# soham2560/MPCHoloNavigation

Hardware: AMD Instinct MI355X
Metric: rollouts/sec per computeVelocityCommands() tick (higher is better)
Workload: dtype f32

## Files before the change

### mpcholonavigation_amd/csrc/smpc_api.cpp

```cpp

#include "smpc_ctx.h"

#include <emmintrin.h>

namespace smpc_impl {

thread_local std::string g_create_error;

int fail(smpc_ctx* c, int code, const std::string& msg)
{
  if (c) c->err = msg; else g_create_error = msg;
  return code;
}

int wait_map_upload(smpc_ctx* c)
{
  if (!c->map_pending) return SMPC_OK;
  HIPCK(c, hipEventSynchronize(c->ev_map));
  c->map_pending = false;
  return SMPC_OK;
}

void bar_copy(void* dev_dst, const void* host_src, size_t n)
{
// ... 291 lines not shown
int update_time_major(smpc_ctx* c)
{
  if (!c->use_tpr) return SMPC_OK;
  const uint32_t B = c->cfg.batch_size, T = c->cfg.time_steps;
  HIPCK(c, smpc_launch_relayout(c->d_nvx, c->d_tvx, B, T, true, c->stream));
  HIPCK(c, smpc_launch_relayout(c->d_nvy, c->d_tvy, B, T, true, c->stream));
  HIPCK(c, smpc_launch_relayout(c->d_nwz, c->d_twz, B, T, true, c->stream));
  return SMPC_OK;
}

int ensure_row_major(smpc_ctx* c)
{
  if (c->rm_valid) return SMPC_OK;
  const uint32_t B = c->cfg.batch_size, T = c->cfg.time_steps;
  HIPCK(c, smpc_launch_relayout(c->d_tvx, c->d_nvx, B, T, false, c->stream));
  if (c->holonomic) HIPCK(c, smpc_launch_relayout(c->d_tvy, c->d_nvy, B, T, false, c->stream));
  HIPCK(c, smpc_launch_relayout(c->d_twz, c->d_nwz, B, T, false, c->stream));
  c->rm_valid = true;
  return SMPC_OK;
}

static int launch_draw(smpc_ctx* c, float* nvx, float* nvy, float* nwz, float* tvx, float* tvy, float* twz,
                       hipStream_t st, bool* rm_valid_out)
{
  const uint64_t n = static_cast<uint64_t>(c->cfg.batch_size) * c->cfg.time_steps;
  const uint64_t base = c->cfg.shard_offset * c->cfg.time_steps;
  const uint32_t B = c->cfg.batch_size, T = c->cfg.time_steps;
  if (c->use_tpr && (T & 3u) == 0 && !getenv("SMPC_NO_FUSED_FILL")) {
    HIPCK(c, smpc_launch_fill_noise_tm(tvx, B, T, base, c->seed, 0, c->epoch, c->cfg.vx_std, st));
    HIPCK(c, smpc_launch_fill_noise_tm(twz, B, T, base, c->seed, 1, c->epoch, c->cfg.wz_std, st));
    if (c->holonomic)
      HIPCK(c, smpc_launch_fill_noise_tm(tvy, B, T, base, c->seed, 2, c->epoch, c->cfg.vy_std, st));
    else
      HIPCK(c, hipMemsetAsync(tvy, 0, static_cast<size_t>(SMPC_GM_ROLLOUTS(B)) * T * sizeof(float), st));
    *rm_valid_out = false;
    return SMPC_OK;
  }
  HIPCK(c, smpc_launch_fill_noise(nvx, n, base, c->seed, 0, c->epoch, c->cfg.vx_std, st));
  HIPCK(c, smpc_launch_fill_noise(nwz, n, base, c->seed, 1, c->epoch, c->cfg.wz_std, st));
  if (c->holonomic) HIPCK(c, smpc_launch_fill_noise(nvy, n, base, c->seed, 2, c->epoch, c->cfg.vy_std, st));
  if (c->use_tpr) {
    HIPCK(c, smpc_launch_relayout(nvx, tvx, B, T, true, st));
    HIPCK(c, smpc_launch_relayout(nvy, tvy, B, T, true, st));
    HIPCK(c, smpc_launch_relayout(nwz, twz, B, T, true, st));
  }
  *rm_valid_out = true;
  return SMPC_OK;
}

int cancel_redraw(smpc_ctx* c)
{
  if (!c->redraw_pending) return SMPC_OK;
  HIPCK(c, hipEventSynchronize(c->ev_fill));
  c->redraw_pending = false;
  return SMPC_OK;
}

int absorb_redraw(smpc_ctx* c)
{
  if (!c->redraw_pending) return SMPC_OK;
  HIPCK(c, hipStreamWaitEvent(c->stream, c->ev_fill, 0));
  std::swap(c->d_nvx, c->b_nvx);
  std::swap(c->d_nvy, c->b_nvy);
  std::swap(c->d_nwz, c->b_nwz);
  std::swap(c->d_tvx, c->b_tvx);
  std::swap(c->d_tvy, c->b_tvy);
  std::swap(c->d_twz, c->b_twz);
  c->rm_valid = c->redraw_rm_valid;
  c->redraw_pending = false;
  c->noise_gen++;
  return SMPC_OK;
}

int draw_noise(smpc_ctx* c)
{
  int rc = cancel_redraw(c);
  if (rc != SMPC_OK) return rc;
  bool rm = true;
  rc = launch_draw(c, c->d_nvx, c->d_nvy, c->d_nwz, c->d_tvx, c->d_tvy, c->d_twz, c->stream, &rm);
  if (rc != SMPC_OK) return rc;
  HIPCK(c, hipStreamSynchronize(c->stream));
  c->have_noise = true;
  c->rm_valid = rm;
  c->noise_gen++;
  return SMPC_OK;
}

int redraw_async(smpc_ctx* c)
{
  if (c->redraw_pending) return SMPC_OK;
  const size_t n = static_cast<size_t>(c->cfg.batch_size) * c->cfg.time_steps * sizeof(float);
  if (!c->fill_stream) {
    HIPCK(c, hipStreamCreateWithFlags(&c->fill_stream, hipStreamNonBlocking));
    HIPCK(c, hipEventCreateWithFlags(&c->ev_fill, hipEventDisableTiming));
  }
  if (c->use_tpr && !c->b_tvx) {
    const size_t ngm = static_cast<size_t>(SMPC_GM_ROLLOUTS(c->cfg.batch_size)) * c->cfg.time_steps * sizeof(float);
    HIPCK(c, hipMalloc(&c->b_tvx, 3 * ngm));
    c->b_tvy = c->b_tvx + ngm / sizeof(float);
    c->b_twz = c->b_tvy + ngm / sizeof(float);
  }
  if (!c->b_nvx) {
    HIPCK(c, hipMalloc(&c->b_nvx, n));
    HIPCK(c, hipMalloc(&c->b_nvy, n));
    HIPCK(c, hipMalloc(&c->b_nwz, n));
    if (!c->holonomic) HIPCK(c, hipMemset(c->b_nvy, 0, n));
  }
  c->epoch++;
  bool rm = true;
  const int rc = launch_draw(c, c->b_nvx, c->b_nvy, c->b_nwz, c->b_tvx, c->b_tvy, c->b_twz, c->fill_stream, &rm);
  if (rc != SMPC_OK) return rc;
  HIPCK(c, hipEventRecord(c->ev_fill, c->fill_stream));
  c->redraw_rm_valid = rm;
  c->redraw_pending = true;
  return SMPC_OK;
}

static Knobs read_knobs()
{
  Knobs k;
  auto set = [](const char* name) {return getenv(name) != nullptr;};
  auto number = [](const char* name, int unset) {const char* e = getenv(name); return e ? atoi(e) : unset;};
  if (const char* e = getenv("SMPC_PASS"))
    k.pass = !strcmp(e, "wave") ? Knobs::kWave : !strcmp(e, "lane") ? Knobs::kLane : !strcmp(e, "split") ? Knobs::kSplit : Knobs::kAuto;
  k.no_split = set("SMPC_NO_SPLIT");
  k.split_nseg = static_cast<uint32_t>(std::max(0, number("SMPC_SPLIT_NSEG", 0)));
  k.lane_reread = number("SMPC_LANE_REREAD", 0) != 0;
  k.half_blocks = !set("SMPC_NO_HALF_BLOCKS");
  k.max_blocks_per_cu = static_cast<uint32_t>(std::max(0, number("SMPC_MAX_BLOCKS_PER_CU", 0)));
  k.balanced_grid = !set("SMPC_NO_BALANCED_GRID");
  k.fused_reduce = set("SMPC_FUSED_REDUCE");
// ... 126 lines not shown
  c->stream = c->own_stream;
  if (getenv("SMPC_LANE_TIMELINE")) {
    static_assert(SMPC_TAIL_STAMPS_AT == 8192 + kMaxGrid * 8, "the tail's stamps sit behind the lane pass's");
    CK(hipMalloc(&c->d_timeline, (SMPC_SCAN_COUNT_AT + kMaxGrid * 8) * sizeof(unsigned long long)));
    CK(hipMemset(c->d_timeline, 0, (SMPC_SCAN_COUNT_AT + kMaxGrid * 8) * sizeof(unsigned long long)));
  }
  CK(hipEventCreate(&c->ev0));
  CK(hipEventCreateWithFlags(&c->ev_map, hipEventDisableTiming));
  CK(hipEventCreate(&c->ev1));
  for (auto& e : c->evp) CK(hipEventCreate(&e));
  const uint32_t T = cfg->time_steps;
  c->R = T <= 64 ? 1 : (T <= 128 ? 2 : 4);
  const size_t n = static_cast<size_t>(cfg->batch_size) * T * sizeof(float);
  CK(hipMalloc(&c->d_nvx, n));
  CK(hipMalloc(&c->d_nvy, n));
  if (!c->holonomic) CK(hipMemset(c->d_nvy, 0, n));
  CK(hipMalloc(&c->d_nwz, n));
  {
    bool tpr = cfg->batch_size >= kLaneMinBatch && cfg->time_steps <= kLaneMaxT;
    if (cfg->time_steps <= 64 && cfg->time_steps >= 36 && (cfg->time_steps & 3u) == 0 && cfg->batch_size >= kSplitMinBatch &&
        !c->knobs.no_split)
      tpr = true;
    if (cfg->flags & SMPC_FLAG_WAVE_PER_ROLLOUT) tpr = false;
    if (cfg->flags & SMPC_FLAG_LANE_PER_ROLLOUT) {
      tpr = true;
      c->lane_forced = true;
    }
    if (c->knobs.pass == Knobs::kWave) tpr = false;
    if (c->knobs.pass == Knobs::kLane || c->knobs.pass == Knobs::kSplit) {
      tpr = true;
      c->lane_forced = true;
    }
    if (cfg->flags & SMPC_FLAG_STORE_TRAJECTORIES) tpr = false;
    const size_t ngm = static_cast<size_t>(SMPC_GM_ROLLOUTS(cfg->batch_size)) * T * sizeof(float);
    if (3ull * ngm >= (1ull << 32)) tpr = false;
    c->use_tpr = tpr;
    if (tpr) {
      CK(hipMalloc(&c->d_tvx, 3 * ngm));
      c->d_tvy = c->d_tvx + ngm / sizeof(float);
      c->d_twz = c->d_tvy + ngm / sizeof(float);
      if (!c->holonomic) CK(hipMemset(c->d_tvy, 0, ngm));
      CK(lane_set_lds_limit(static_cast<int>(kLdsPerCu)));
      CK(split_set_lds_limit(static_cast<int>(kLdsPerCu)));
    }
  }
  CK(hipMalloc(&c->d_costs[0], cfg->batch_size * sizeof(float)));
  CK(hipMalloc(&c->d_costs[1], cfg->batch_size * sizeof(float)));
  CK(hipMemset(c->d_costs[0], 0, cfg->batch_size * sizeof(float)));
  CK(hipMemset(c->d_costs[1], 0, cfg->batch_size * sizeof(float)));
  if (cfg->flags & SMPC_FLAG_STORE_TRAJECTORIES) {
    for (int i = 0; i < 3; ++i) {
      CK(hipMalloc(&c->d_traj[i], n));
      CK(hipMemset(c->d_traj[i], 0, n));
    }
  }
  c->tick_cap = tick_layout(T, SMPC_MAX_PATH).total;
  CK(hipMalloc(&c->d_tick, c->tick_cap));
  CK(hipHostMalloc(&c->h_tick, c->tick_cap, hipHostMallocDefault));
  CK(hipMalloc(&c->d_lut, 256 * sizeof(SmpcLut)));
  CK(hipMemset(c->d_lut, 0, 256 * sizeof(SmpcLut)));
  CK(hipMalloc(&c->d_lut_fp, 512 * sizeof(SmpcLut)));
  CK(hipMemset(c->d_lut_fp, 0, 512 * sizeof(SmpcLut)));
  CK(hipHostMalloc(&c->h_lut_fp, 512 * sizeof(SmpcLut), hipHostMallocDefault));
  CK(hipHostMalloc(&c->h_lut, 256 * sizeof(SmpcLut), hipHostMallocDefault));
  const size_t TL = 4 + 3 * static_cast<size_t>(T);
  CK(hipMalloc(&c->d_partials, (kMaxGrid * TL + 16) * sizeof(float)));
  CK(hipMemset(c->d_partials, 0, (kMaxGrid * TL + 16) * sizeof(float)));
  CK(hipMalloc(&c->d_tuple, TL * sizeof(float)));
  CK(hipMalloc(&c->d_out, (3 * T + 8) * sizeof(float)));
  CK(hipMalloc(&c->d_u_iter, 3 * T * sizeof(float)));
  CK(hipHostMalloc(&c->h_out, (3 * T + 8 + kPollWords) * sizeof(float), hipHostMallocMapped));
  memset(c->h_out, 0, (3 * T + 8 + kPollWords) * sizeof(float));
  CK(hipHostGetDevicePointer(reinterpret_cast<void**>(&c->h_out_dev), c->h_out, 0));
  CK(hipMalloc(&c->d_furthest, 32));
// ... 605 lines not shown
```

### mpcholonavigation_amd/csrc/smpc_dev.h

```cpp
#ifndef SMPC_DEV_H_
#define SMPC_DEV_H_

#include <stdint.h>

#define SD_OBSTACLES 0x001u
#define SD_PATH_ALIGN 0x002u
#define SD_PATH_FOLLOW 0x004u
#define SD_GOAL_ANGLE 0x008u
#define SD_PREFER_FORWARD 0x010u
#define SD_USE_PATH_YAW 0x020u
#define SD_ACCUMULATE 0x040u
#define SD_STORE_TRAJ 0x080u
#define SD_TRACK_UNKNOWN 0x100u
#define SD_NEED_FURTHEST 0x200u
#define SD_LOCAL_FURTHEST 0x400u
#define SD_CONSTRAINT 0x800u
#define SD_COST 0x1000u
#define SD_GOAL 0x2000u
#define SD_TWIRLING 0x4000u
#define SD_PATH_ANGLE 0x8000u
#define SD_DEADBAND 0x10000u
#define SD_FP_OBSTACLES 0x20000u
#define SD_FP_COST 0x40000u
#define SD_PATH_ALIGN_LEGACY 0x80000u
#define SD_PAL_USE_PATH_YAW 0x100000u
#define SD_EXTRA_CRITICS (SD_CONSTRAINT | SD_COST | SD_GOAL | SD_TWIRLING | SD_PATH_ANGLE | SD_DEADBAND | \
                          SD_FP_OBSTACLES | SD_FP_COST | SD_PATH_ALIGN_LEGACY)

#define SMPC_GM_ROLLOUTS(B) ((((B) + 63u) / 64u) * 64u)
#define SMPC_GM_INDEX(b, t, T) ((((size_t)(b) >> 6) * (T) + (t)) * 64u + ((b) & 63u))

#define SMPC_MAX_PATH 1024
#define SMPC_MAX_R 4

struct SmpcLut {
  float crit;
  float rep;
};

struct SmpcFinal {
  int enabled;
  float vx_max, vx_min, vy_max, wz_max;
  float* u_dev;
  float* u_host;
  const float* furthest_used;
  uint32_t* done_counter;
  uint32_t seq;
};

struct SmpcDev {
  uint32_t B, T, P;
  uint32_t nsamp;
  uint32_t step;
  uint32_t flags;
  double x0, y0;
  float yaw0, cos0, sin0;
  float svx, svy, swz;
  float dt;
  const float* nvx;
  const float* nvy;
  const float* nwz;
  const float* tvx;
  const float* tvy;
// ... 174 lines not shown
```

### mpcholonavigation_amd/csrc/smpc_kernels.hip

```cpp

#include <hip/hip_runtime.h>
#include <stdio.h>
#include <algorithm>
#include <stdint.h>

#include "smpc_dev.h"
#include "smpc_device_math.h"
#include "smpc_tail.h"
#include "smpc_inst.h"

#define WAVE 64

template <int CTRL, int ROW_MASK = 0xF>
__device__ __forceinline__ float dpp_f(float old, float v)
{
  return __int_as_float(__builtin_amdgcn_update_dpp(__float_as_int(old), __float_as_int(v), CTRL,
                                                    ROW_MASK, 0xF, false));
}
template <int CTRL, int ROW_MASK = 0xF>
__device__ __forceinline__ uint32_t dpp_u(uint32_t old, uint32_t v)
{
  return (uint32_t)__builtin_amdgcn_update_dpp((int)old, (int)v, CTRL, ROW_MASK, 0xF, false);
}

// ... 1308 lines not shown
                                                      float sigma)
{
  const uint64_t q_first = base >> 2;
  const uint64_t q_last = (base + n + 3) >> 2;
  for (uint64_t q = q_first + (uint64_t)blockIdx.x * blockDim.x + threadIdx.x; q < q_last;
       q += (uint64_t)gridDim.x * blockDim.x) {
    uint32_t r[4];
    philox4x32_10((uint32_t)q, (uint32_t)(q >> 32), stream, epoch, (uint32_t)seed,
                  (uint32_t)(seed >> 32), r);
    float z[4];
    box_muller(r[0], r[1], z[0], z[1]);
    box_muller(r[2], r[3], z[2], z[3]);
    const uint64_t e0 = q << 2;
#pragma unroll
    for (int k = 0; k < 4; ++k) {
      const uint64_t e = e0 + (uint64_t)k;
      if (e >= base && e < base + n) out[e - base] = z[k] * sigma;
    }
  }
}

__global__ void __launch_bounds__(256) smpc_fill_noise_tm(float* __restrict__ dst, uint32_t B, uint32_t T,
                                                         uint64_t base, uint64_t seed, uint32_t stream,
                                                         uint32_t epoch, float sigma)
{
  const uint32_t tq = blockIdx.y;
  for (uint32_t b = blockIdx.x * blockDim.x + threadIdx.x; b < B; b += gridDim.x * blockDim.x) {
    const uint64_t q = (base + (uint64_t)b * T + 4u * tq) >> 2;
    uint32_t r[4];
    philox4x32_10((uint32_t)q, (uint32_t)(q >> 32), stream, epoch, (uint32_t)seed, (uint32_t)(seed >> 32), r);
    float z[4];
    box_muller(r[0], r[1], z[0], z[1]);
    box_muller(r[2], r[3], z[2], z[3]);
#pragma unroll
    for (int k = 0; k < 4; ++k) dst[SMPC_GM_INDEX(b, 4u * tq + (uint32_t)k, T)] = z[k] * sigma;
  }
}

__global__ void smpc_sincos_kernel(const float* __restrict__ x, uint32_t n,
                                   float* __restrict__ sn, float* __restrict__ cs)
{
  const uint32_t i = blockIdx.x * blockDim.x + threadIdx.x;
  if (i < n) {
    float s, c;
    smpc_sincos(x[i], s, c);
    sn[i] = s;
    cs[i] = c;
  }
}

hipError_t smpc_launch_sincos(const float* x, uint32_t n, float* sn, float* cs, hipStream_t st)
{
  hipLaunchKernelGGL(smpc_sincos_kernel, dim3((n + 255) / 256), dim3(256), 0, st, x, n, sn, cs);
  return hipGetLastError();
}

__global__ void smpc_philox_kernel(const uint32_t* __restrict__ ctr, uint32_t k0, uint32_t k1, uint32_t n,
                                   uint32_t* __restrict__ out)
{
  const uint32_t i = blockIdx.x * blockDim.x + threadIdx.x;
  if (i < n) {
    uint32_t r[4];
    philox4x32_10(ctr[4 * i], ctr[4 * i + 1], ctr[4 * i + 2], ctr[4 * i + 3], k0, k1, r);
#pragma unroll
    for (int k = 0; k < 4; ++k) out[4 * i + k] = r[k];
  }
}

// ... 139 lines not shown
```

### mpcholonavigation_amd/csrc/smpc_lane.hip

```cpp

#include <hip/hip_runtime.h>
#include <stdint.h>
#include <stdio.h>

#include <type_traits>

#include "smpc_dev.h"
#include "smpc_device_math.h"
#include "smpc_tail.h"
#include "smpc_lane_common.h"
#include "smpc_inst.h"

#ifndef WAVE
#define WAVE 64
#endif
#define LANE_BLOCK 512
#define LANE_BLOCK_RR 512

template <bool TO_GM>
__global__ void __launch_bounds__(256) smpc_relayout(const float* __restrict__ src, float* __restrict__ dst,
                                                    uint32_t B, uint32_t T)
{
  __shared__ float tile[32][33];
  const uint32_t b0 = blockIdx.x * 32, t0 = blockIdx.y * 32;
  const uint32_t lx = threadIdx.x & 31, ly = threadIdx.x >> 5;
  if (TO_GM) {
    for (uint32_t k = ly; k < 32; k += 8) {
      const uint32_t b = b0 + k, t = t0 + lx;
      tile[k][lx] = (b < B && t < T) ? src[(size_t)b * T + t] : 0.f;
    }
    __syncthreads();
    for (uint32_t k = ly; k < 32; k += 8) {
      const uint32_t t = t0 + k, b = b0 + lx;
      if (b < B && t < T) dst[SMPC_GM_INDEX(b, t, T)] = tile[lx][k];
    }
  } else {
    for (uint32_t k = ly; k < 32; k += 8) {
      const uint32_t t = t0 + k, b = b0 + lx;
      tile[lx][k] = (b < B && t < T) ? src[SMPC_GM_INDEX(b, t, T)] : 0.f;
    }
    __syncthreads();
    for (uint32_t k = ly; k < 32; k += 8) {
      const uint32_t b = b0 + k, t = t0 + lx;
      if (b < B && t < T) dst[(size_t)b * T + t] = tile[k][lx];
    }
  }
}

hipError_t smpc_launch_relayout(const float* src, float* dst, uint32_t B, uint32_t T, bool to_gm, hipStream_t st)
{
  const dim3 grid((B + 31) / 32, (T + 31) / 32);
  if (to_gm) hipLaunchKernelGGL(smpc_relayout<true>, grid, dim3(256), 0, st, src, dst, B, T);
  else hipLaunchKernelGGL(smpc_relayout<false>, grid, dim3(256), 0, st, src, dst, B, T);
  return hipGetLastError();
}

__global__ void __launch_bounds__(64) smpc_lane_reduce_kernel(const float* __restrict__ v,
                                                              const float* __restrict__ w,
                                                              float* __restrict__ out)
{
  const int lane = threadIdx.x;
  float V[64];
#pragma unroll
  for (int t = 0; t < 64; ++t) V[t] = v[lane * 64 + t];
  const LaneW lw = lane_weights(w[lane], lane);
  out[lane] = lane_reduce64(V, lw, lane);
}

hipError_t smpc_launch_lane_reduce(const float* v, const float* w, float* out, hipStream_t st)
{
  hipLaunchKernelGGL(smpc_lane_reduce_kernel, dim3(1), dim3(64), 0, st, v, w, out);
  return hipGetLastError();
// ... 132 lines not shown
```

### mpcholonavigation_amd/csrc/smpc_lane_pass.inc

```
template <bool FULL, bool OBST, bool MANY, int NCH, bool RR, bool GA = false, bool QUADS = FULL, int TC = 0, bool DEP = false>
__global__ void __launch_bounds__(RR ? LANE_BLOCK_RR : LANE_BLOCK, 1)
LANE_PASS_KERNEL(const SmpcDev p0, const SmpcLds L, const SmpcDev* __restrict__ many)
{
  constexpr bool POW = LANE_PASS_POW;
  constexpr bool NH = LANE_PASS_NH;
  static_assert(!NH || (OBST && !MANY && !RR && !GA && !DEP && !POW && NCH == 1 && QUADS),
                "no vy stream: the plain ObstaclesCritic rows of whole quads only");
  static_assert(RR || NCH == 1, "parked controls: one chunk of 64 steps");
  static_assert(!POW || (!MANY && !RR && !DEP), "cost powers: the single-context parking form of the five critics");
  static_assert(!FULL || QUADS, "T == 64 is a multiple of four");
  static_assert(TC == 0 || (!FULL && QUADS && !RR && TC < 64 && (TC & 3) == 0), "compile-time horizon: whole quads below 64");
  static_assert(!DEP || (OBST && !RR && !GA), "deployed-list instances: parking form");
  const SmpcDev& p = MANY ? many[blockIdx.y] : p0;
  const SmpcTickPtrs tk{p.u, p.px, p.py, p.pyaw, p.D, p.pf_idx, p.pvalid, p.pa_active, p.pang_active, p.pal_active};
  extern __shared__ __attribute__((aligned(16))) unsigned char smem[];
  uint8_t* s_map = smem;
  const SmpcLut* s_lut = reinterpret_cast<const SmpcLut*>(smem + L.off_lut);
  float* s_px = reinterpret_cast<float*>(smem + L.off_px);
  float* s_py = reinterpret_cast<float*>(smem + L.off_py);
  float* s_D = reinterpret_cast<float*>(smem + L.off_D) + 1;
  f32x4* s_pts4 = reinterpret_cast<f32x4*>(smem + L.off_pts4);
  float* s_su2 = reinterpret_cast<float*>(smem + L.off_scr) - 4;
  constexpr bool kPrune = !GA && !DEP && !MANY && !RR && !POW;
  float* s_prune = reinterpret_cast<float*>(smem + L.off_prune);
// ... 64 lines not shown
      float a = 0.f, b = 0.f, c = 0.f;
      const uint32_t Tn = FULL ? 64u * NCH : (TC ? (uint32_t)TC : p.T);
      for (uint32_t t = (uint32_t)tid; t < Tn; t += WAVE) {
        const float ux = tk.u[t], uy = NH ? 0.f : tk.u[Tn + t], uz = tk.u[2 * Tn + t];
        a = fmaf(ux, ux, a);
        b = fmaf(uy, uy, b);
        c = fmaf(uz, uz, c);
      }
      for (int o = 32; o > 0; o >>= 1) {
        a += __shfl_xor(a, o, WAVE);
        b += __shfl_xor(b, o, WAVE);
        c += __shfl_xor(c, o, WAVE);
      }
      if (tid == 0) {
        s_su2[0] = a;
        s_su2[1] = b;
        s_su2[2] = c;
      }
    }
    for (uint32_t i = tid + blk; i < p.P; i += blk) {
      const float qx = tk.px[i], qy = tk.py[i];
      const bool seg = i + 1 < p.P;
      s_px[i] = qx;
      s_py[i] = qy;
      if (seg) s_D[i] = tk.D[i];
      s_pts4[i] = f32x4{qx, qy, (seg && tk.pvalid[i]) ? 1.0f : 0.f, 0.f};
    }
  }
  __syncthreads();
  stamp(1);

  const cfloat_p cu = (cfloat_p)(uintptr_t)p.u;
  const uint32_t T = FULL ? 64u * NCH : (TC ? (uint32_t)TC : p.T), B = p.B;
  const uint32_t noise_bytes = T * SMPC_GM_ROLLOUTS(B) * 4u;
  const __amdgpu_buffer_rsrc_t rn = __builtin_amdgcn_make_buffer_rsrc(const_cast<float*>(p.tvx), 0, 3u * noise_bytes, 0x00020000);
  const float dt = p.dt, yaw0 = p.yaw0;
  const double x0 = p.x0, y0 = p.y0;
  uint32_t S = 0;
  if (p.flags & SD_NEED_FURTHEST) {
    S = p.d_furthest ? smpc_furthest_index(*p.d_furthest) : p.furthest_hint;
    if (S >= p.P) S = p.P ? p.P - 1 : 0;
  }
  if (lane == 0) {
    s_D[-1] = -3.0e38f;
    s_D[S] = 3.0e38f;
  }
  const bool pa_on = (p.flags & SD_PATH_ALIGN) && p.P > 0 && tk.pa_active[S] && S > 0;
  float pf_x = 0.f, pf_y = 0.f;
  if ((p.flags & SD_PATH_FOLLOW) && p.P > 0) {
    const uint32_t idx = tk.pf_idx[S];
    pf_x = tk.px[idx];
    pf_y = tk.py[idx];
  }
  const uint32_t bs_iters = S > 1 ? 32u - (uint32_t)__builtin_clz(S - 1) : 0u;
  float pa_inv_spacing = 0.f;
  if (pa_on && S > 1 && tk.D[S - 1] > 0.f) pa_inv_spacing = (float)(S - 1) / tk.D[S - 1];
  const bool want_local_furthest = (p.flags & SD_NEED_FURTHEST) && (p.flags & SD_LOCAL_FURTHEST);
  const bool con_on = DEP && (p.flags & SD_CONSTRAINT) != 0, tw_on = DEP && (p.flags & SD_TWIRLING) != 0;
  const float k_con = p.dt * p.con_weight, k_tw = p.tw_weight / (float)(FULL ? 64 * NCH : (TC ? TC : (int)p.T));
  const bool cost_mode = DEP && (p.flags & SD_COST) != 0;
  constexpr bool ga_on = GA;
  const uint32_t nquad = (T + 3u) >> 2;

  float m_run = 3.0e38f, s_run = 0.f;
  float Ux[NCH], Uy[NCH], Uz[NCH];
#pragma unroll
  for (int h = 0; h < NCH; ++h) Ux[h] = Uy[h] = Uz[h] = 0.f;
// ... 13 lines not shown
    const bool live = b < B;
    const uint32_t bl = live ? b : B - 1;
    f32x32 PX0, PX1, PY0, PY1;
    if constexpr (NH) {
      if (!FULL) PX0 = PX1 = (f32x32)(0.f);
    } else if (!FULL && !RR) PX0 = PX1 = PY0 = PY1 = (f32x32)(0.f);

    float cpx = p.svx, cpy = NH ? 0.f : p.svy, cpz = p.swz;
    float acc_yaw = 0.f, ax = 0.f, ay = 0.f;
    float cs_prev = p.cos0, sn_prev = p.sin0;
    float x = 0.f, y = 0.f;
    float crit = 0.f, rep = 0.f;
    float yaw_max = 0.f;
    float alive = 1.0f;
    uint32_t cell_q = 256u;
    f32x2 e_q = {0.f, 0.f};
    auto lookup_wait = [&]() {};
    auto lookup_accumulate = [&]() {
      alive = e_q.x < 0.f ? 0.f : alive;
      crit = fmaf(alive, e_q.x, crit);
      rep = fmaf(alive, e_q.y, rep);
    };
    auto lookup_issue_entry = [&]() {
      const SmpcLut e = s_lut[cell_q];
      e_q = f32x2{e.crit, e.rep};
    };
    auto lookup_issue_byte = [&](uint32_t idx) {cell_q = s_map[idx];};
    float pfw = 0.f, gx = 0.f, gy = 0.f, gz = 0.f;
    float ga_sum = 0.f;
    float ext = 0.f;
    float traj_dist = 0.f, pa_sum = 0.f, pa_num = 0.f, sx_prev = p.x00f, sy_prev = p.y00f;
    uint32_t path_pt = 0;

    const float k_rinv = p.rinvf, k_cx = p.cxf, k_cy = p.cyf;
    const float k_edge = 0.5f - p.cell_eps_w;
    auto do_step = [&](const uint32_t t, const bool sample_slot, const float ux, const float uy, const float uz,
                       const float n0, const float n1, const float n2, float& cvx, float& cvy,
                       float& cwz) __attribute__((always_inline)) {
      cvx = ux + n0;
      if constexpr (!NH) cvy = uy + n1;
      cwz = uz + n2;
      const float vx = cpx, vy = cpy, wz = cpz;
      cpx = cvx;
      if constexpr (!NH) cpy = cvy;
      cpz = cwz;
      acc_yaw = acc_yaw + wz * dt;
      const float yaw = acc_yaw + yaw0;
      const float dxr = NH ? vx * cs_prev : vx * cs_prev - vy * sn_prev;
      const float dyr = NH ? vx * sn_prev : vx * sn_prev + vy * cs_prev;
      ax = ax + dxr * dt;
      ay = ay + dyr * dt;
      if constexpr (DEP) {
        if (con_on) {
          const float sp = fast_sqrt(vx * vx + vy * vy);
          const float vt = vx > 0.f ? sp : -sp;
          const float e = fmaxf(vt - p.con_max_vel, 0.f) + fmaxf(p.con_min_vel - vt, 0.f);
          ext = fmaf(e, k_con, ext);
        }
        if (tw_on) ext = fmaf(fabsf(wz), k_tw, ext);
      }
      if (ga_on) {
        const float a = p.ga_goal_yaw - yaw;
        const float kf = fmaf(a, 0.15915494309189535f, 12582912.0f);
        const float k = kf - 12582912.0f;
        float r = fmaf(-k, 6.2831854820251465f, a);
        r = fmaf(-k, -1.7484555e-07f, r);
        ga_sum += fabsf(r);
      }

      uint32_t idx = 0;
      if (OBST) {
        const float qx = fmaf(ax, k_rinv, k_cx), qy = fmaf(ay, k_rinv, k_cy);
        const float rx = __builtin_amdgcn_fractf(qx), ry = __builtin_amdgcn_fractf(qy);
        const int lx = cvt_floor_i32(qx), ly = cvt_floor_i32(qy);
// ... 36 lines not shown
        uint32_t lo = gi + (c1 ? 1u : 0u);
        float dl = c1 ? db : da, dh = c1 ? dc : db;
        if (__builtin_expect(__builtin_amdgcn_ballot_w64(!c0 || c2) != 0, 0)) {
          uint32_t base = 0, nn = S;
          for (uint32_t it = 0; it < bs_iters; ++it) {
            const uint32_t half = nn >> 1;
            base = (s_D[base + half - 1 + (half == 0)] < dist && half) ? base + half : base;
            nn -= half;
          }
          const float d_base = s_D[base];
          lo = base + (d_base < dist ? 1u : 0u);
          dl = lo > 0 ? s_D[lo - 1] : 0.f;
          dh = lo < S ? s_D[lo] : 0.f;
        }
        uint32_t pt;
        if (lo == path_pt) pt = 0;
        else if (lo >= S) pt = S - 1;
        else pt = (dist - dl < dh - dist) ? lo - 1 : lo;
        path_pt = pt;
        const f32x4 q = s_pts4[pt];
        const float ex = q[0] - x, ey = q[1] - y;
        const float d = fast_sqrt(ex * ex + ey * ey);
        pa_num += q[2];
        pa_sum = fmaf(q[2], d, pa_sum);
      }
      if (OBST) {
        lookup_wait();
        lookup_accumulate();
        lookup_issue_entry();
        lookup_issue_byte(idx);
      }
    };

    const uint32_t loff = ((bl >> 6) * T * 64u + (bl & 63u)) * 4u;
    constexpr uint32_t step_bytes = 256u;
    auto ld = [&](uint32_t tensor, uint32_t t) -> float {
      const uint32_t tc = (FULL || t < T) ? t : T - 1;
      return __uint_as_float(__builtin_amdgcn_raw_buffer_load_b32(rn, loff, tensor * noise_bytes + tc * step_bytes, 0));
    };
    auto ldu = [&](uint32_t ctrl, uint32_t t) -> float {return cu[ctrl * T + ((FULL || t < T) ? t : T - 1)];};
    float nq[12], uq[12];
#pragma unroll
    for (int i = 0; i < 4; ++i) {
      nq[3 * i + 0] = ld(0, i);
      if constexpr (!NH) nq[3 * i + 1] = ld(1, i);
      nq[3 * i + 2] = ld(2, i);
#pragma unroll
      for (int k = 0; k < 3; ++k) {
        if constexpr (NH) {
          if (k == 1) continue;
        }
        uq[3 * i + k] = ldu(k, i);
      }
    }
    uint64_t clk = __builtin_amdgcn_s_memtime();
    auto run_quad = [&](auto hi_c, auto swap_c, const uint32_t q, float (&cq)[12]) __attribute__((always_inline)) {
      constexpr bool SWAP = decltype(swap_c)::value;
      if constexpr (SWAP) {
        __builtin_amdgcn_s_setprio(0);
        if (((uint32_t)(clk >> 15) + (uint32_t)(wave >> 2)) & 1u) __builtin_amdgcn_s_setprio(1);
        clk = __builtin_amdgcn_s_memtime();
      }
      float uc[12];
#pragma unroll
      for (int j = 0; j < 12; ++j) {
        if constexpr (NH) {
          if (j % 3 == 1) continue;
        }
        uc[j] = uq[j];
      }
      constexpr bool kAlwaysAhead = !FULL && TC == 0;
      if (kAlwaysAhead || q + 1 < nquad) {
#pragma unroll
        for (int i = 0; i < 4; ++i)
#pragma unroll
          for (int k = 0; k < 3; ++k) {
            if constexpr (NH) {
              if (k == 1) continue;
            }
            uq[3 * i + k] = ldu(k, 4 * (q + 1) + i);
          }
      }
      constexpr bool kQuadOff = QUADS && !GA && !DEP && !MANY && !POW;
#pragma unroll
      for (int i = 0; i < 4; ++i) {
        const uint32_t t = 4 * q + i;
        const float n0 = nq[3 * i], n1 = NH ? 0.f : nq[3 * i + 1], n2 = nq[3 * i + 2];
        if (kAlwaysAhead || q + 1 < nquad) {
          if constexpr (kQuadOff) {
            const uint32_t tq = (FULL || TC || 4 * (q + 1) < T) ? 4 * (q + 1) : T - 4;
            const uint32_t so0 = tq * step_bytes, so1 = noise_bytes + so0, so2 = noise_bytes + so1;
            auto ldq = [&](uint32_t so) -> float {
              return __uint_as_float(__builtin_amdgcn_raw_buffer_load_b32(rn, loff + (uint32_t)i * step_bytes, so, 0));
            };
            nq[3 * i + 0] = ldq(so0);
            if constexpr (!NH) nq[3 * i + 1] = ldq(so1);
            nq[3 * i + 2] = ldq(so2);
          } else {
            nq[3 * i + 0] = ld(0, t + 4);
            nq[3 * i + 1] = ld(1, t + 4);
            nq[3 * i + 2] = ld(2, t + 4);
          }
        }
        cq[3 * i] = cq[3 * i + 1] = cq[3 * i + 2] = 0.f;
        if (QUADS || t < T)
          do_step(t, i == 0, uc[3 * i], NH ? 0.f : uc[3 * i + 1], uc[3 * i + 2], n0, n1, n2, cq[3 * i], cq[3 * i + 1],
                  cq[3 * i + 2]);
      }
    };
    constexpr bool kPairLoops = FULL || TC != 0;
#define LANE_PARK_QUAD(HI, Q) \
      if constexpr (!RR) { \
        _Pragma("unroll") for (int i = 0; i < 4; ++i) { \
          if constexpr (HI) { \
            PX1[8 * i + ((Q) - 8)] = cq[3 * i]; \
            if constexpr (!NH) PY1[8 * i + ((Q) - 8)] = cq[3 * i + 1]; \
          } else { \
            PX0[8 * i + (Q)] = cq[3 * i]; \
            if constexpr (!NH) PY0[8 * i + (Q)] = cq[3 * i + 1]; \
          } \
          park[(4 * (Q) + i) * LANE_PARK_STRIDE + lane] = cq[3 * i + 2]; \
        } \
      }
    if constexpr (kPairLoops) {
#define LANE_QUAD(HI, SWAP, Q) \
    { \
      float cq[12]; \
      run_quad(std::bool_constant<HI>{}, std::bool_constant<SWAP>{}, (Q), cq); \
      LANE_PARK_QUAD(HI, Q) \
    }
#define LANE_QUADS(HI, Q0, QE)    \
    { \
      uint32_t q = (Q0); \
      const uint32_t qe = (QE); \
      for (; q + 1 < qe; q += 2) { \
        LANE_QUAD(HI, true, q) \
        LANE_QUAD(HI, false, q + 1) \
// ... 117 lines not shown
        uni += p.pf_weight * fast_sqrt(fdx * fdx + fdy * fdy);
      }
      if (p.flags & SD_PREFER_FORWARD) lin += (pfw * -dt) * p.pfw_weight;
      if (ga_on) uni += (ga_sum / (float)T) * p.ga_weight;
      lin += p.g_vx * (gx - s_su2[0]);
      lin += p.g_wz * (gz - s_su2[2]);
      if constexpr (!NH) lin += p.g_vy * (gy - s_su2[1]);
      cost += uni + lin;
      if (pa_on) {
        const float c_pa = pa_num > 0.f ? pa_sum * fast_rcp(pa_num) : 0.f;
        cost += c_pa * p.pa_weight;
      }
    }
    if (live) p.costs[b] = cost;

    float cmin = live ? cost : 3.0e38f;
    for (int o = 32; o > 0; o >>= 1) cmin = fminf(cmin, __shfl_xor(cmin, o, WAVE));
    const float m_new = fminf(m_run, cmin);
    const float f = __builtin_amdgcn_exp2f(p.k2 * (m_run - m_new));
    const float w = live ? __builtin_amdgcn_exp2f(p.k2 * (cost - m_new)) : 0.f;
    float wsum = w;
    for (int o = 32; o > 0; o >>= 1) wsum += __shfl_xor(wsum, o, WAVE);
    s_run = fmaf(s_run, f, wsum);
    m_run = m_new;

    const LaneW lw = lane_weights(w, lane);
    if constexpr (RR) {
#pragma unroll
      for (int h = 0; h < NCH; ++h) {
#pragma unroll
        for (int ctrl = 0; ctrl < 3; ++ctrl) {
          float V[64];
#pragma unroll
          for (int t = 0; t < 64; ++t) V[t] = ld(ctrl, 64u * h + t);
          __builtin_amdgcn_sched_barrier(0);
#pragma unroll
          for (int t = 0; t < 64; ++t) {
            const uint32_t tt = 64u * h + t;
            const float c = ldu(ctrl, tt) + V[t];
            V[t] = (FULL || tt < T) ? c : 0.f;
          }
          const float r = lane_reduce64(V, lw, lane);
          if (ctrl == 0) Ux[h] = fmaf(Ux[h], f, r);
          else if (ctrl == 1) Uy[h] = fmaf(Uy[h], f, r);
          else Uz[h] = fmaf(Uz[h], f, r);
        }
      }
    } else {
      {
        float V[64];
#pragma unroll
        for (int t = 0; t < 32; ++t) {
          V[t] = PX0[8 * (t & 3) + (t >> 2)];
          V[32 + t] = PX1[8 * (t & 3) + (t >> 2)];
        }
        Ux[0] = fmaf(Ux[0], f, lane_reduce64(V, lw, lane));
        if constexpr (!NH) {
#pragma unroll
          for (int t = 0; t < 32; ++t) {
            V[t] = PY0[8 * (t & 3) + (t >> 2)];
            V[32 + t] = PY1[8 * (t & 3) + (t >> 2)];
          }
          Uy[0] = fmaf(Uy[0], f, lane_reduce64(V, lw, lane));
        }
      }
      {
        s_w[lane] = w;
// ... 84 lines not shown
```

### mpcholonavigation_amd/csrc/smpc_split.hip

```cpp

#include <hip/hip_runtime.h>
#include <stdint.h>
#include <stdio.h>

#include "smpc_dev.h"
#include "smpc_device_math.h"
#include "smpc_lane_common.h"
#include "smpc_inst.h"

#define SPLIT_BLOCK 512

typedef const float __attribute__((address_space(4))) * cfloat_ps;
typedef float f32x16 __attribute__((ext_vector_type(16)));
typedef float f32x8 __attribute__((ext_vector_type(8)));
template <int N> struct vecN;
template <> struct vecN<32> {typedef f32x32 type;};
template <> struct vecN<16> {typedef f32x16 type;};
template <> struct vecN<8> {typedef f32x8 type;};
template <> struct vecN<4> {typedef f32x4 type;};

template <int N, int K, int Rr>
__device__ __forceinline__ float row_reduce_node(const float (&V)[N], int lane)
{
  if constexpr ((64 >> K) == N) {
// ... 134 lines not shown
      if (seg_on) s_D[tid] = g_D;
      s_pts4[tid] = f32x4{g_px, g_py, g_valid ? 1.0f : 0.f, 0.f};
    }
    for (uint32_t i = tid + blk; i < p.P; i += blk) {
      const float qx = tk.px[i], qy = tk.py[i];
      const bool seg = i + 1 < p.P;
      s_px[i] = qx;
      s_py[i] = qy;
      if (seg) s_D[i] = tk.D[i];
      s_pts4[i] = f32x4{qx, qy, (seg && tk.pvalid[i]) ? 1.0f : 0.f, 0.f};
    }
    if (tid < 3 * 64) s_u[tid] = g_u;
    if (tid < WAVE) {
      const bool in = (uint32_t)tid < T;
      float a = in ? tk.u[tid] : 0.f, b = in ? tk.u[T + tid] : 0.f, c = in ? tk.u[2 * T + tid] : 0.f;
      a *= a;
      b *= b;
      c *= c;
      for (int o = 32; o > 0; o >>= 1) {
        a += __shfl_xor(a, o, WAVE);
        b += __shfl_xor(b, o, WAVE);
        c += __shfl_xor(c, o, WAVE);
      }
      if (tid == 0) {
        s_su2[0] = a;
        s_su2[1] = b;
        s_su2[2] = c;
      }
    }
  }
  __syncthreads();

  const uint32_t B = p.B;
  const uint32_t noise_bytes = T * SMPC_GM_ROLLOUTS(B) * 4u;
  const __amdgpu_buffer_rsrc_t rn = __builtin_amdgcn_make_buffer_rsrc(const_cast<float*>(p.tvx), 0, 3u * noise_bytes, 0x00020000);
  constexpr uint32_t row_bytes = 256u;
  const float dt = p.dt, yaw0 = p.yaw0;
  const double x0 = p.x0, y0 = p.y0;
  uint32_t S = 0;
  if (p.flags & SD_NEED_FURTHEST) {
    S = p.d_furthest ? smpc_furthest_index(*p.d_furthest) : p.furthest_hint;
    if (S >= p.P) S = p.P ? p.P - 1 : 0;
  }
  if (lane == 0) {
    s_D[-1] = -3.0e38f;
    s_D[S] = 3.0e38f;
  }
  const bool pa_on = (p.flags & SD_PATH_ALIGN) && p.P > 0 && tk.pa_active[S] && S > 0;
  float pf_x = 0.f, pf_y = 0.f;
  if ((p.flags & SD_PATH_FOLLOW) && p.P > 0) {
    const uint32_t idx = tk.pf_idx[S];
    pf_x = tk.px[idx];
    pf_y = tk.py[idx];
  }
  const uint32_t bs_iters = S > 1 ? 32u - (uint32_t)__builtin_clz(S - 1) : 0u;
  float pa_inv_spacing = 0.f;
  if (pa_on && S > 1 && tk.D[S - 1] > 0.f) pa_inv_spacing = (float)(S - 1) / tk.D[S - 1];
  const bool want_local_furthest = (p.flags & SD_NEED_FURTHEST) && (p.flags & SD_LOCAL_FURTHEST);
  const float k_rinv = p.rinvf, k_cx = p.cxf, k_cy = p.cyf;
  const float k_edge = 0.5f - p.cell_eps_w;

  float m_run = 3.0e38f, s_run = 0.f;
  float Ux = 0.f, Uy = 0.f, Uz = 0.f;
  float F_local = 0.f;
  uint32_t n_noncoll = 0;

  const uint32_t ngroups = (B + SPLIT_ROLL - 1) / SPLIT_ROLL;
  const uint32_t gw = blockIdx.x * nwave + wave;
  const uint32_t nW = gridDim.x * nwave;
  const uint32_t t0 = (uint32_t)sg * SPLIT_SEG;

  for (uint32_t grp = gw; grp < ngroups; grp += nW) {
    const uint32_t b = grp * SPLIT_ROLL + (uint32_t)r;
    const bool live = b < B;
    const uint32_t bl = live ? b : B - 1;
    const uint32_t voff = ((bl >> 6) * T * 64u + (bl & 63u)) * 4u + t0 * row_bytes;
    const uint32_t vprev = sg ? voff - row_bytes : voff;
    auto ld = [&](uint32_t tensor, uint32_t i) -> float {
      return __uint_as_float(__builtin_amdgcn_raw_buffer_load_b32(rn, voff, tensor * noise_bytes + i * row_bytes, 0));
    };
    auto ld_prev = [&](uint32_t tensor) -> float {
      return __uint_as_float(__builtin_amdgcn_raw_buffer_load_b32(rn, vprev, tensor * noise_bytes, 0));
    };
    const float* ux_s = s_u + t0;
    const float* uy_s = s_u + 64 + t0;
    const float* uz_s = s_u + 128 + t0;
    auto act = [&](int i) -> bool {return FULL || t0 + (uint32_t)i < T;};

    float ya[SPLIT_SEG];
    float wprev;
    {
      float nz[SPLIT_SEG];
      const float nzp = ld_prev(2);
#pragma unroll
      for (int i = 0; i < SPLIT_SEG; ++i) nz[i] = ld(2, i);
      const float uzp = s_u[128 + (sg ? t0 - 1 : 0)];
      wprev = sg ? uzp + nzp : p.swz;
      float acc = 0.f, w = wprev;
#pragma unroll
      for (int i = 0; i < SPLIT_SEG; ++i) {
        acc = acc + w * dt;
        ya[i] = acc;
        w = act(i) ? uz_s[i] + nz[i] : 0.f;
        park[i * WAVE + lane] = w;
      }
    }
    const float yaw_off = seg_exclusive<NSEG>(ya[SPLIT_SEG - 1], r, sg);

    constexpr int Q = SPLIT_SEG / 4;
#define SLOT(i) (Q * ((i) & 3) + ((i) >> 2))
    typename vecN<SPLIT_SEG>::type cvx;
    float cvy[PARK_VY ? 1 : SPLIT_SEG];
    typename vecN<SPLIT_SEG>::type AX, AY;
    float vxp, vyp;
    {
      const float nxp = ld_prev(0), nyp = ld_prev(1);
      float ny[SPLIT_SEG];
#pragma unroll
      for (int i = 0; i < SPLIT_SEG; ++i) {
        cvx[SLOT(i)] = ld(0, i);
        ny[i] = ld(1, i);
      }
      vxp = sg ? s_u[t0 - 1] + nxp : p.svx;
      vyp = sg ? s_u[64 + t0 - 1] + nyp : p.svy;
#pragma unroll
      for (int i = 0; i < SPLIT_SEG; ++i) {
        cvx[SLOT(i)] = act(i) ? ux_s[i] + cvx[SLOT(i)] : 0.f;
        ny[i] = act(i) ? uy_s[i] + ny[i] : 0.f;
        if constexpr (PARK_VY) park_y[i * WAVE + lane] = ny[i];
        else cvy[i] = ny[i];
      }
      float cs_prev = p.cos0, sn_prev = p.sin0;
      if (sg) smpc_sincos(yaw_off + yaw0, sn_prev, cs_prev);
      float ax = 0.f, ay = 0.f;
#pragma unroll
      for (int i = 0; i < SPLIT_SEG; ++i) {
        const float vx = i ? cvx[SLOT(i - 1)] : vxp, vy = i ? ny[i - 1] : vyp;
        const float dxr = vx * cs_prev - vy * sn_prev;
        const float dyr = vx * sn_prev + vy * cs_prev;
        ax = ax + dxr * dt;
        ay = ay + dyr * dt;
        AX[SLOT(i)] = ax;
        AY[SLOT(i)] = ay;
        if (i + 1 < SPLIT_SEG) smpc_sincos((yaw_off + ya[i]) + yaw0, sn_prev, cs_prev);
      }
    }
    const float x_off = seg_exclusive<NSEG>(AX[SLOT(SPLIT_SEG - 1)], r, sg);
    const float y_off = seg_exclusive<NSEG>(AY[SLOT(SPLIT_SEG - 1)], r, sg);

    float crit = 0.f, rep = 0.f, alive = 1.0f;
    float pfw = 0.f, gx = 0.f, gy = 0.f, gz = 0.f;
    typename vecN<NSAMP>::type sxv, syv;
    float x_end = 0.f, y_end = 0.f;
    float vx_state = vxp;
// ... 338 lines not shown
```

Baseline: 5.765 billion.

## Interleave noise tensors in groups of four timesteps for 128-bit loads

```diff
diff --git a/mpcholonavigation_amd/csrc/smpc_api.cpp b/mpcholonavigation_amd/csrc/smpc_api.cpp
--- a/mpcholonavigation_amd/csrc/smpc_api.cpp
+++ b/mpcholonavigation_amd/csrc/smpc_api.cpp
@@ -347,7 +347,7 @@
     if (c->holonomic)
       HIPCK(c, smpc_launch_fill_noise_tm(tvy, B, T, base, c->seed, 2, c->epoch, c->cfg.vy_std, st));
     else
-      HIPCK(c, hipMemsetAsync(tvy, 0, static_cast<size_t>(SMPC_GM_ROLLOUTS(B)) * T * sizeof(float), st));
+      HIPCK(c, hipMemsetAsync(tvy, 0, SMPC_GM_ELEMS(B, T) * sizeof(float), st));
     *rm_valid_out = false;
     return SMPC_OK;
   }
@@ -410,8 +410,9 @@
     HIPCK(c, hipEventCreateWithFlags(&c->ev_fill, hipEventDisableTiming));
   }
   if (c->use_tpr && !c->b_tvx) {
-    const size_t ngm = static_cast<size_t>(SMPC_GM_ROLLOUTS(c->cfg.batch_size)) * c->cfg.time_steps * sizeof(float);
+    const size_t ngm = SMPC_GM_ELEMS(c->cfg.batch_size, c->cfg.time_steps) * sizeof(float);
     HIPCK(c, hipMalloc(&c->b_tvx, 3 * ngm));
+    HIPCK(c, hipMemset(c->b_tvx, 0, 3 * ngm));
     c->b_tvy = c->b_tvx + ngm / sizeof(float);
     c->b_twz = c->b_tvy + ngm / sizeof(float);
   }
@@ -604,14 +605,14 @@
       c->lane_forced = true;
     }
     if (cfg->flags & SMPC_FLAG_STORE_TRAJECTORIES) tpr = false;
-    const size_t ngm = static_cast<size_t>(SMPC_GM_ROLLOUTS(cfg->batch_size)) * T * sizeof(float);
+    const size_t ngm = SMPC_GM_ELEMS(cfg->batch_size, T) * sizeof(float);
     if (3ull * ngm >= (1ull << 32)) tpr = false;
     c->use_tpr = tpr;
     if (tpr) {
       CK(hipMalloc(&c->d_tvx, 3 * ngm));
       c->d_tvy = c->d_tvx + ngm / sizeof(float);
       c->d_twz = c->d_tvy + ngm / sizeof(float);
-      if (!c->holonomic) CK(hipMemset(c->d_tvy, 0, ngm));
+      CK(hipMemset(c->d_tvx, 0, 3 * ngm));
       CK(lane_set_lds_limit(static_cast<int>(kLdsPerCu)));
       CK(split_set_lds_limit(static_cast<int>(kLdsPerCu)));
     }
diff --git a/mpcholonavigation_amd/csrc/smpc_dev.h b/mpcholonavigation_amd/csrc/smpc_dev.h
--- a/mpcholonavigation_amd/csrc/smpc_dev.h
+++ b/mpcholonavigation_amd/csrc/smpc_dev.h
@@ -28,7 +28,10 @@
                           SD_FP_OBSTACLES | SD_FP_COST | SD_PATH_ALIGN_LEGACY)
 
 #define SMPC_GM_ROLLOUTS(B) ((((B) + 63u) / 64u) * 64u)
-#define SMPC_GM_INDEX(b, t, T) ((((size_t)(b) >> 6) * (T) + (t)) * 64u + ((b) & 63u))
+#define SMPC_GM_STEPS(T) (((T) + 3u) & ~3u)
+#define SMPC_GM_ELEMS(B, T) ((size_t)SMPC_GM_ROLLOUTS(B) * SMPC_GM_STEPS(T))
+#define SMPC_GM_INDEX(b, t, T) \
+  (((((size_t)(b) >> 6) * (SMPC_GM_STEPS(T) >> 2) + ((t) >> 2)) * 64u + ((b) & 63u)) * 4u + ((t) & 3u))
 
 #define SMPC_MAX_PATH 1024
 #define SMPC_MAX_R 4
diff --git a/mpcholonavigation_amd/csrc/smpc_kernels.hip b/mpcholonavigation_amd/csrc/smpc_kernels.hip
--- a/mpcholonavigation_amd/csrc/smpc_kernels.hip
+++ b/mpcholonavigation_amd/csrc/smpc_kernels.hip
@@ -1364,8 +1364,9 @@
     float z[4];
     box_muller(r[0], r[1], z[0], z[1]);
     box_muller(r[2], r[3], z[2], z[3]);
-#pragma unroll
-    for (int k = 0; k < 4; ++k) dst[SMPC_GM_INDEX(b, 4u * tq + (uint32_t)k, T)] = z[k] * sigma;
+    typedef float fill_f32x4 __attribute__((ext_vector_type(4)));
+    *reinterpret_cast<fill_f32x4*>(dst + SMPC_GM_INDEX(b, 4u * tq, T)) =
+        fill_f32x4{z[0] * sigma, z[1] * sigma, z[2] * sigma, z[3] * sigma};
   }
 }
 
diff --git a/mpcholonavigation_amd/csrc/smpc_lane.hip b/mpcholonavigation_amd/csrc/smpc_lane.hip
--- a/mpcholonavigation_amd/csrc/smpc_lane.hip
+++ b/mpcholonavigation_amd/csrc/smpc_lane.hip
@@ -31,13 +31,15 @@
     }
     __syncthreads();
     for (uint32_t k = ly; k < 32; k += 8) {
-      const uint32_t t = t0 + k, b = b0 + lx;
-      if (b < B && t < T) dst[SMPC_GM_INDEX(b, t, T)] = tile[lx][k];
+      const uint32_t e = k * 32 + lx, tl = 4 * (e >> 7) + (e & 3), bb = (e >> 2) & 31;
+      const uint32_t t = t0 + tl, b = b0 + bb;
+      if (b < B && t < T) dst[SMPC_GM_INDEX(b, t, T)] = tile[bb][tl];
     }
   } else {
     for (uint32_t k = ly; k < 32; k += 8) {
-      const uint32_t t = t0 + k, b = b0 + lx;
-      tile[lx][k] = (b < B && t < T) ? src[SMPC_GM_INDEX(b, t, T)] : 0.f;
+      const uint32_t e = k * 32 + lx, tl = 4 * (e >> 7) + (e & 3), bb = (e >> 2) & 31;
+      const uint32_t t = t0 + tl, b = b0 + bb;
+      tile[bb][tl] = (b < B && t < T) ? src[SMPC_GM_INDEX(b, t, T)] : 0.f;
     }
     __syncthreads();
     for (uint32_t k = ly; k < 32; k += 8) {
diff --git a/mpcholonavigation_amd/csrc/smpc_lane_pass.inc b/mpcholonavigation_amd/csrc/smpc_lane_pass.inc
--- a/mpcholonavigation_amd/csrc/smpc_lane_pass.inc
+++ b/mpcholonavigation_amd/csrc/smpc_lane_pass.inc
@@ -120,7 +120,8 @@
 
   const cfloat_p cu = (cfloat_p)(uintptr_t)p.u;
   const uint32_t T = FULL ? 64u * NCH : (TC ? (uint32_t)TC : p.T), B = p.B;
-  const uint32_t noise_bytes = T * SMPC_GM_ROLLOUTS(B) * 4u;
+  const uint32_t T4 = SMPC_GM_STEPS(T);
+  const uint32_t noise_bytes = (uint32_t)SMPC_GM_ELEMS(B, T) * 4u;
   const __amdgpu_buffer_rsrc_t rn = __builtin_amdgcn_make_buffer_rsrc(const_cast<float*>(p.tvx), 0, 3u * noise_bytes, 0x00020000);
   const float dt = p.dt, yaw0 = p.yaw0;
   const double x0 = p.x0, y0 = p.y0;
@@ -200,14 +201,19 @@
     float traj_dist = 0.f, pa_sum = 0.f, pa_num = 0.f, sx_prev = p.x00f, sy_prev = p.y00f;
     uint32_t path_pt = 0;
 
-    const float k_rinv = p.rinvf, k_cx = p.cxf, k_cy = p.cyf;
+    constexpr bool kCellVgpr = OBST && QUADS && (FULL || TC != 0) && !GA && !DEP && !MANY && !RR && !POW;
+    const float k_rinv = p.rinvf, k_cx = kCellVgpr ? in_vgpr(p.cxf) : p.cxf, k_cy = kCellVgpr ? in_vgpr(p.cyf) : p.cyf;
     const float k_edge = 0.5f - p.cell_eps_w;
+    constexpr bool kAddAtTop = FULL && !RR && (GA || (MANY && DEP));
+    constexpr int kFetchAt = GA ? 3 : 1;
     auto do_step = [&](const uint32_t t, const bool sample_slot, const float ux, const float uy, const float uz,
                        const float n0, const float n1, const float n2, float& cvx, float& cvy,
                        float& cwz) __attribute__((always_inline)) {
-      cvx = ux + n0;
-      if constexpr (!NH) cvy = uy + n1;
-      cwz = uz + n2;
+      if constexpr (!kAddAtTop) {
+        cvx = ux + n0;
+        if constexpr (!NH) cvy = uy + n1;
+        cwz = uz + n2;
+      }
       const float vx = cpx, vy = cpy, wz = cpz;
       cpx = cvx;
       if constexpr (!NH) cpy = cvy;
@@ -310,19 +316,20 @@
       }
     };
 
-    const uint32_t loff = ((bl >> 6) * T * 64u + (bl & 63u)) * 4u;
-    constexpr uint32_t step_bytes = 256u;
-    auto ld = [&](uint32_t tensor, uint32_t t) -> float {
-      const uint32_t tc = (FULL || t < T) ? t : T - 1;
-      return __uint_as_float(__builtin_amdgcn_raw_buffer_load_b32(rn, loff, tensor * noise_bytes + tc * step_bytes, 0));
+    const uint32_t loff = (bl >> 6) * (T4 * 256u) + (bl & 63u) * 16u;
+    constexpr uint32_t quad_bytes = 1024u;
+    auto ldq = [&](uint32_t tensor, uint32_t q) -> f32x4 {
+      const uint32_t qc = (FULL || TC || q < nquad) ? q : nquad - 1;
+      return __builtin_bit_cast(f32x4, __builtin_amdgcn_raw_buffer_load_b128(rn, loff, tensor * noise_bytes + qc * quad_bytes, 0));
     };
     auto ldu = [&](uint32_t ctrl, uint32_t t) -> float {return cu[ctrl * T + ((FULL || t < T) ? t : T - 1)];};
-    float nq[12], uq[12];
+    f32x4 nq0, nq1, nq2;
+    float uq[12];
+    nq0 = ldq(0, 0);
+    if constexpr (!NH) nq1 = ldq(1, 0);
+    nq2 = ldq(2, 0);
 #pragma unroll
     for (int i = 0; i < 4; ++i) {
-      nq[3 * i + 0] = ld(0, i);
-      if constexpr (!NH) nq[3 * i + 1] = ld(1, i);
-      nq[3 * i + 2] = ld(2, i);
 #pragma unroll
       for (int k = 0; k < 3; ++k) {
         if constexpr (NH) {
@@ -359,28 +366,35 @@
             uq[3 * i + k] = ldu(k, 4 * (q + 1) + i);
           }
       }
-      constexpr bool kQuadOff = QUADS && !GA && !DEP && !MANY && !POW;
+      const f32x4 nc0 = nq0, nc1 = NH ? (f32x4)(0.f) : nq1, nc2 = nq2;
+      if constexpr (kAddAtTop) {
+#pragma unroll
+        for (int i = 0; i < 4; ++i) {
+          cq[3 * i] = uc[3 * i] + nc0[i];
+          cq[3 * i + 1] = uc[3 * i + 1] + nc1[i];
+          cq[3 * i + 2] = uc[3 * i + 2] + nc2[i];
+        }
+      }
+      auto fetch = [&]() __attribute__((always_inline)) {
+        if (kAlwaysAhead || q + 1 < nquad) {
+          nq0 = ldq(0, q + 1);
+          if constexpr (!NH) nq1 = ldq(1, q + 1);
+          nq2 = ldq(2, q + 1);
+        }
+      };
+      if constexpr (!kAddAtTop) fetch();
 #pragma unroll
       for (int i = 0; i < 4; ++i) {
         const uint32_t t = 4 * q + i;
-        const float n0 = nq[3 * i], n1 = NH ? 0.f : nq[3 * i + 1], n2 = nq[3 * i + 2];
-        if (kAlwaysAhead || q + 1 < nquad) {
-          if constexpr (kQuadOff) {
-            const uint32_t tq = (FULL || TC || 4 * (q + 1) < T) ? 4 * (q + 1) : T - 4;
-            const uint32_t so0 = tq * step_bytes, so1 = noise_bytes + so0, so2 = noise_bytes + so1;
-            auto ldq = [&](uint32_t so) -> float {
-              return __uint_as_float(__builtin_amdgcn_raw_buffer_load_b32(rn, loff + (uint32_t)i * step_bytes, so, 0));
-            };
-            nq[3 * i + 0] = ldq(so0);
-            if constexpr (!NH) nq[3 * i + 1] = ldq(so1);
-            nq[3 * i + 2] = ldq(so2);
-          } else {
-            nq[3 * i + 0] = ld(0, t + 4);
-            nq[3 * i + 1] = ld(1, t + 4);
-            nq[3 * i + 2] = ld(2, t + 4);
+        if constexpr (kAddAtTop) {
+          if (i == kFetchAt) {
+            __builtin_amdgcn_sched_barrier(0);
+            fetch();
+            __builtin_amdgcn_sched_barrier(0);
           }
         }
-        cq[3 * i] = cq[3 * i + 1] = cq[3 * i + 2] = 0.f;
+        const float n0 = nc0[i], n1 = nc1[i], n2 = nc2[i];
+        if constexpr (!kAddAtTop) cq[3 * i] = cq[3 * i + 1] = cq[3 * i + 2] = 0.f;
         if (QUADS || t < T)
           do_step(t, i == 0, uc[3 * i], NH ? 0.f : uc[3 * i + 1], uc[3 * i + 2], n0, n1, n2, cq[3 * i], cq[3 * i + 1],
                   cq[3 * i + 2]);
@@ -564,7 +578,11 @@
         for (int ctrl = 0; ctrl < 3; ++ctrl) {
           float V[64];
 #pragma unroll
-          for (int t = 0; t < 64; ++t) V[t] = ld(ctrl, 64u * h + t);
+          for (int j = 0; j < 16; ++j) {
+            const f32x4 v = ldq(ctrl, 16u * h + j);
+#pragma unroll
+            for (int e = 0; e < 4; ++e) V[4 * j + e] = v[e];
+          }
           __builtin_amdgcn_sched_barrier(0);
 #pragma unroll
           for (int t = 0; t < 64; ++t) {
diff --git a/mpcholonavigation_amd/csrc/smpc_split.hip b/mpcholonavigation_amd/csrc/smpc_split.hip
--- a/mpcholonavigation_amd/csrc/smpc_split.hip
+++ b/mpcholonavigation_amd/csrc/smpc_split.hip
@@ -190,9 +190,9 @@
   __syncthreads();
 
   const uint32_t B = p.B;
-  const uint32_t noise_bytes = T * SMPC_GM_ROLLOUTS(B) * 4u;
+  const uint32_t noise_bytes = (uint32_t)SMPC_GM_ELEMS(B, T) * 4u;
   const __amdgpu_buffer_rsrc_t rn = __builtin_amdgcn_make_buffer_rsrc(const_cast<float*>(p.tvx), 0, 3u * noise_bytes, 0x00020000);
-  constexpr uint32_t row_bytes = 256u;
+  constexpr uint32_t quad_bytes = 1024u;
   const float dt = p.dt, yaw0 = p.yaw0;
   const double x0 = p.x0, y0 = p.y0;
   uint32_t S = 0;
@@ -232,10 +232,10 @@
     const uint32_t b = grp * SPLIT_ROLL + (uint32_t)r;
     const bool live = b < B;
     const uint32_t bl = live ? b : B - 1;
-    const uint32_t voff = ((bl >> 6) * T * 64u + (bl & 63u)) * 4u + t0 * row_bytes;
-    const uint32_t vprev = sg ? voff - row_bytes : voff;
-    auto ld = [&](uint32_t tensor, uint32_t i) -> float {
-      return __uint_as_float(__builtin_amdgcn_raw_buffer_load_b32(rn, voff, tensor * noise_bytes + i * row_bytes, 0));
+    const uint32_t voff = (bl >> 6) * (T * 256u) + (bl & 63u) * 16u + (t0 >> 2) * quad_bytes;
+    const uint32_t vprev = sg ? voff - quad_bytes + 12u : voff;
+    auto ldq = [&](uint32_t tensor, uint32_t j) -> f32x4 {
+      return __builtin_bit_cast(f32x4, __builtin_amdgcn_raw_buffer_load_b128(rn, voff, tensor * noise_bytes + j * quad_bytes, 0));
     };
     auto ld_prev = [&](uint32_t tensor) -> float {
       return __uint_as_float(__builtin_amdgcn_raw_buffer_load_b32(rn, vprev, tensor * noise_bytes, 0));
@@ -251,7 +251,11 @@
       float nz[SPLIT_SEG];
       const float nzp = ld_prev(2);
 #pragma unroll
-      for (int i = 0; i < SPLIT_SEG; ++i) nz[i] = ld(2, i);
+      for (int j = 0; j < SPLIT_SEG / 4; ++j) {
+        const f32x4 v = ldq(2, j);
+#pragma unroll
+        for (int e = 0; e < 4; ++e) nz[4 * j + e] = v[e];
+      }
       const float uzp = s_u[128 + (sg ? t0 - 1 : 0)];
       wprev = sg ? uzp + nzp : p.swz;
       float acc = 0.f, w = wprev;
@@ -275,9 +279,13 @@
       const float nxp = ld_prev(0), nyp = ld_prev(1);
       float ny[SPLIT_SEG];
 #pragma unroll
-      for (int i = 0; i < SPLIT_SEG; ++i) {
-        cvx[SLOT(i)] = ld(0, i);
-        ny[i] = ld(1, i);
+      for (int j = 0; j < SPLIT_SEG / 4; ++j) {
+        const f32x4 vx4 = ldq(0, j), vy4 = ldq(1, j);
+#pragma unroll
+        for (int e = 0; e < 4; ++e) {
+          cvx[SLOT(4 * j + e)] = vx4[e];
+          ny[4 * j + e] = vy4[e];
+        }
       }
       vxp = sg ? s_u[t0 - 1] + nxp : p.svx;
       vyp = sg ? s_u[64 + t0 - 1] + nyp : p.svy;
```

After: 5.992 billion (median of 6 runs). 4.0% higher.
